# yvette256/nerfstudio-thermal

Measured on AMD Instinct MI355X. Metric: train rays/sec (4096-ray batch, 96 samples/ray), higher is better.
Workload: dtype f32; 1 GPU; thermal-nerfacto density_mode=shared train step (pixel sampling+raygen+fwd+losses+bwd+allreduce+Adam), 4096 rays/GPU, 256/96 proposal + 48 field samples, hash 16x2^19x2 + 2x(5x2^17x2), 8 cameras (4 RGB + 4 thermal); rays_per_gpu=4096, parallelism=dp1, grad_scaler=device-side (optim.DeviceGradScaler)

## Files before the change

### nerfstudio-thermal_amd/csrc/tn_adam.h

```cpp
#pragma once
#include "tn_common.h"

struct AdamCoef {
  float neg_step, bc2_sqrt;
  float b1, b2, omb1, omb2, eps;
};
__host__ __device__ __forceinline__ AdamCoef adam_coef(float neg_step, float bc2_sqrt, double beta1, double beta2, float eps) {
  return AdamCoef{neg_step, bc2_sqrt, (float)beta1, (float)beta2, (float)(1.0 - beta1), (float)(1.0 - beta2), eps};
}
__device__ __forceinline__ void adam1(float& p, float g, float& m, float& v, const AdamCoef& c) {
  const float m_new = m * c.b1 + g * c.omb1;
  const float v_new = v * c.b2 + (c.omb2 * g) * g;
  const float den = sqrtf(v_new) / c.bc2_sqrt + c.eps;
  p = p + c.neg_step * (m_new / den);
  m = m_new;
  v = v_new;
}
#pragma clang fp contract(off)
__device__ __forceinline__ double adam_bias_correction(double beta, int step, int skipped) {
  const int eff = step - skipped;
  return 1.0 - pow(beta, (double)(eff < 1 ? 1 : eff));
}
__device__ __forceinline__ double adam_sched_t(int max_steps, int sched_step, int lag) {
  const double t = (double)(sched_step - lag) / (double)max_steps;
// ... 19 lines not shown
#define TN_FOLD_ADAM_FUSED 1.0f
#define TN_FOLD_ADAM_FELL_BACK 2.0f
struct FoldAdamHost {
  float *p, *m, *v;
  float* state;
  float* found_inf;
  int flag;
  const int32_t* skipped;
  int lag_index;
  int step, max_steps, sched_step;
  double lr, lr_final, beta1, beta2;
  float eps;
  const float* grads;
  int ncheck;
  int64_t check_off[TN_TRAIN_STEP_MAX_RANGES], check_cnt[TN_TRAIN_STEP_MAX_RANGES];
};
```

### nerfstudio-thermal_amd/csrc/tn_common.h

```cpp
#pragma once
#include <hip/hip_runtime.h>
#include <stdint.h>
#include <math.h>
#include "../../include/thermal_nerf_hip.h"

#define TN_WAVE 64

void tn_set_error(const char* fmt, ...);
#define TN_REQUIRE(cond, ...)        \
  do {                               \
    if (!(cond)) {                   \
      tn_set_error(__VA_ARGS__);     \
      return TN_EINVAL;              \
    }                                \
  } while (0)
#define TN_CHECK_LAUNCH(name)                                         \
  do {                                                                \
    hipError_t e__ = hipGetLastError();                               \
    if (e__ != hipSuccess) {                                          \
      tn_set_error("%s: %s", name, hipGetErrorString(e__));           \
      return TN_ELAUNCH;                                              \
    }                                                                 \
  } while (0)

// ... 350 lines not shown
int tn_train_losses_clip(const float* s_bins_fine, const float* weights_fine, int32_t S_fine, int32_t num_props, const float* const* s_bins_prop,
                         const float* const* weights_prop, const int32_t* S_prop, float* const* d_weights_prop, int64_t N, float distortion_mult,
                         float interlevel_mult, float* d_weights_fine, const float* pred_rgb, int32_t rgb_stride, const float* pred_thermal,
                         int32_t thermal_stride, const float* image, const float* is_thermal, float thermal_mult, float tv_mult, float cross_mult,
                         float* d_pred_rgb, float* d_pred_thermal, float* loss_lines, float* depth_expected, const float* scratch, int clip_nblk,
                         tn_stream_t stream);
struct DposArgs;
struct PoseFinishArgs;
struct FoldAdamHost;
int tn_grid_scatter_launch(const TnGrid& grid, const float* origins, const float* directions, const float* e_bins, const float* g_enc, int ld,
                           int64_t N, int S, float* d_origins, float* d_directions, void* scratch, hipStream_t stream, float* dense_sum = nullptr,
                           bool counters_zeroed = false, const DposArgs* cowork = nullptr, const PoseFinishArgs* fold_cowork = nullptr,
                           const FoldAdamHost* fold_adam = nullptr);
bool tn_grid_scatter_takes_cowork(const TnGrid& grid, int64_t P, void* scratch);
bool tn_fold_adam_takes(const TnGrid& grid, int64_t P, void* scratch);
int tn_field_bwd_phase_ex(const TnField* field, const float* origins, const float* directions, const int64_t* camera_indices, const float* e_bins,
                          const float* d_density, const float* d_rgb, int64_t N, int32_t S, void* workspace, int64_t workspace_bytes, float* d_origins,
                          float* d_directions, int32_t phases, int32_t level_begin, int32_t level_end, const PoseFinishArgs* fold_cowork,
                          bool* fold_cowork_taken, tn_stream_t stream, const FoldAdamHost* fold_adam = nullptr);
int tn_pose_finish_args(const float* pose_adjustment, const uint8_t* frozen, const int64_t* camera_indices, const float* directions_in,
                        const float* d_origins, const float* d_directions, int64_t N, int32_t num_cameras, float* grad_pose, const float* loss_lines,
                        float* losses16, float trans_pen, float rot_pen, float scale, float* reg_out, const float* grads, int32_t num_ranges,
                        const int64_t* offsets, const int64_t* counts, const int32_t* flag_index, int32_t num_flags, float* found_inf, int32_t pose_flag,
                        PoseFinishArgs& a);
void tn_grid_scatter_counters(const TnGrid& grid, int64_t P, void* scratch, uint32_t** ptr, int* words);
__device__ __forceinline__ void tn_zero_words(uint32_t* __restrict__ p, int words) {
  if (blockIdx.x == 0 && blockIdx.y == 0)
    for (int i = threadIdx.x; i < words; i += blockDim.x) p[i] = 0u;
}
bool tn_grid_scatter_is_binned(const TnGrid& grid, int64_t P, const void* scratch);
// ... 8 lines not shown
```

### nerfstudio-thermal_amd/csrc/tn_field.hip

```cpp
#include "tn_common.h"
#include "tn_field_dpos.h"
#include <stdlib.h>

typedef float f32x16 __attribute__((ext_vector_type(16)));
typedef float v4f_t __attribute__((ext_vector_type(4)));
#ifndef FRAG_NT
#define FRAG_NT 1
#endif

#define TILE 32
#define FRAG 64

__host__ __device__ __forceinline__ constexpr int RROW(int r, int h) { return (r & 3) + 8 * (r >> 2) + 4 * h; }

struct LayerGeom { int mo, ti; };
__host__ __device__ __forceinline__ constexpr int layer_mo(int l) { return (l == 0 || l == 2 || l == 3) ? 2 : 1; }
__host__ __device__ __forceinline__ constexpr int layer_ti(int l) { return l == 0 ? 1 : 2; }
__host__ __device__ __forceinline__ constexpr int layer_frags(int l) { return layer_mo(l) * layer_ti(l) * 16; }
__host__ __device__ __forceinline__ constexpr int fwd_off(int l) {
  int o = 0;
  for (int i = 0; i < l; ++i) o += layer_frags(i) * FRAG;
  return o;
}
#define PACK_FWD_FLOATS (fwd_off(5))
// ... 770 lines not shown
#define FB_NO_SB 0
#endif
#ifndef FB_TOUCH
#define FB_TOUCH 0
#endif
#define FB_SB() do { if (!FB_NO_SB) __builtin_amdgcn_sched_barrier(0); } while (0)
template <bool DENS_ONLY, bool BF3>
__global__ void __launch_bounds__(256, 1) k_field_bwd_fused(const float* __restrict__ pack, const float* __restrict__ sel, const float* __restrict__ ys,
                                                            const float* __restrict__ d_rgb, const float* __restrict__ d_density,
                                                            const int64_t* __restrict__ cam_idx, int num_images, int64_t P, int S, int C,
                                                            const float* __restrict__ shtab, const float* __restrict__ emb,
                                                            float* __restrict__ cam_bias, int L, int64_t PT,
                                                            const float* __restrict__ encs, const float* __restrict__ h1s,
                                                            const float* __restrict__ hins, const float* __restrict__ hh1s,
                                                            const float* __restrict__ hh2s, float* __restrict__ g_enc, FusedGrads G,
                                                            uint32_t* __restrict__ zero_ptr, int zero_words) {
  extern __shared__ __attribute__((aligned(16))) float lds[];
  tn_zero_words(zero_ptr, zero_words);
  const float* src = pack + PACK_BWD_OFF;
  for (int i = threadIdx.x * 4; i < PACK_BWD_FLOATS; i += blockDim.x * 4) {
    const float* sp = (BF3 && i >= fwd_off(2) && i < fwd_off(4)) ? pack + PACK_BF_BWD_OFF + (i - fwd_off(2)) : src + i;
    *reinterpret_cast<float4*>(lds + i) = *reinterpret_cast<const float4*>(sp);
  }
  __syncthreads();
  const int lane = threadIdx.x & 63, j = lane & 31, h = lane >> 5, wv = threadIdx.x >> 6;
  float* bufY = lds + PACK_BWD_FLOATS + wv * FB_WAVE_FLOATS;
  float* bufX = bufY + FB_TILE_FLOATS;
  float* bufG = bufX + FB_TILE_FLOATS;
  int* bufC = reinterpret_cast<int*>(bufG + 128);
  const int64_t ntiles = tn_cdiv(P, TILE);
  const int64_t wave = (int64_t)blockIdx.x * 4 + wv;
// ... 14 lines not shown
#pragma unroll
  for (int b = 0; b < 4; ++b) { acc4[b] = zero4; acc1[b] = zero4; }
  int emb_cam = -1;
  float emb_sum = 0.0f;
  const int64_t tpw = tn_cdiv(ntiles, nwaves);
  const int64_t tile_begin = wave * tpw;
  const int64_t tile_end = (wave + 1) * tpw < ntiles ? (wave + 1) * tpw : ntiles;
  f32x16 nx0 = zero16, nx1 = zero16;
  FbSmall nsm;
  if (tile_begin < tile_end) {
    nsm = fb_load_small<DENS_ONLY>(tile_begin, tile_begin, j, h, P, S, C, num_images, hins, d_density, sel, ys, d_rgb, cam_idx);
    nx0 = load_frag(DENS_ONLY ? h1s : hh2s, tile_begin, 2, 0, lane);
    nx1 = load_frag(DENS_ONLY ? h1s : hh2s, tile_begin, 2, 1, lane);
  }
  float touch_acc = 0.0f;
  for (int64_t tile = tile_begin; tile < tile_end; ++tile) {
    const int64_t p = tile * TILE + j;
    const bool valid = p < P;
    const int64_t pc = valid ? p : P - 1;
    const FbSmall sm = nsm;
    float tch0 = 0.0f, tch1 = 0.0f, tch2 = 0.0f;
    if (FB_TOUCH && tile + 1 < tile_end) {
      const int64_t tn = tile + 1;
      if (!DENS_ONLY) tch0 = hh1s[(tn * 2 * 4 * 64) * 4 + lane * 32];
      tch1 = h1s[(tn * 2 * 4 * 64) * 4 + lane * 32];
      if (lane < 16) {
        if (!DENS_ONLY) tch2 = hins[(tn * 128) * 4 + lane * 32];
      } else if (lane < 48) {
        const int l = (lane - 16) >> 1;
        if (l < L) tch2 = encs[((int64_t)l * PT + tn * TILE) * 2 + ((lane - 16) & 1) * 32];
// ... 126 lines not shown
    }
    WAVE_LDS_SYNC();
    if (!(FB_ABLATE & 2)) wgrad_tile32<2, 1>(bufY, bufX, j, h, acc0, bs0);
    FB_SB();
    f32x16 de = zero16;
#pragma unroll
    for (int r = 0; r < 16; ++r) de = MFMA(AB(0, 0, 0, r), dh0[r], de);
#pragma unroll
    for (int r = 0; r < 16; ++r) de = MFMA(AB(0, 0, 1, r), dh1[r], de);
    if (valid) {
#pragma unroll
      for (int g = 0; g < 4; ++g) {
        *reinterpret_cast<float2*>(g_enc + (int64_t)(4 * g + 2 * h) * 2 * P + 2 * p) = make_float2(de[4 * g], de[4 * g + 1]);
        *reinterpret_cast<float2*>(g_enc + (int64_t)(4 * g + 2 * h + 1) * 2 * P + 2 * p) = make_float2(de[4 * g + 2], de[4 * g + 3]);
      }
    }
    WAVE_LDS_SYNC();
    touch_acc += (tch0 + tch1) + tch2;
  }
#undef AB
  if (touch_acc == 1.2345678e-30f) cam_bias[0] = touch_acc;
  if (FB_ABLATE & 8) return;
  __syncthreads();
  float* red = lds + PACK_BWD_FLOATS;
  if (!DENS_ONLY) {
    float* esum = red + FB_RED_TOTAL;
    int* ecam = reinterpret_cast<int*>(esum + 4 * 64);
    esum[wv * 64 + lane] = emb_sum;
    if (lane == 0) ecam[wv] = emb_cam;
    __syncthreads();
    if (threadIdx.x < 64) {
      for (int e = 0; e < 4; ++e) {
        const int cam = ecam[e];
        if (cam < 0) continue;
        bool first = true;
        for (int f = 0; f < e; ++f) first = first && (ecam[f] != cam);
// ... 248 lines not shown
             "tn_field_bwd: bad phase set %d", phases);
  TN_REQUIRE(!((phases & TN_BWD_SCATTER) && (phases & (TN_BWD_SCATTER_BIN | TN_BWD_SCATTER_FOLD))), "tn_field_bwd: TN_BWD_SCATTER and its two halves exclude each other");
  if (phases & (TN_BWD_SCATTER | TN_BWD_SCATTER_FOLD))
    TN_REQUIRE(level_begin >= 0 && level_begin < level_end && level_end <= field->grid.num_levels, "tn_field_bwd: bad level range [%d, %d)", level_begin,
               level_end);
  int64_t P = N * (int64_t)S;
  FieldWs ws = ws_layout(workspace, P, 1);
  TN_REQUIRE(workspace_bytes >= ws.bytes, "tn_field_bwd: workspace of %lld bytes, tn_field_workspace_bytes(%lld, 1) = %lld", (long long)workspace_bytes, (long long)P,
             (long long)ws.bytes);
  TN_REQUIRE((2 * ws.PT + P) * 8 < (1ll << 32), "tn_field_bwd: batch too large for the 32-bit lane offsets of the level-major loads");
  hipStream_t st = tn_s(stream);
  const int C = field->num_channels;
  TN_REQUIRE(dens_only || !(phases & TN_BWD_MLP) || field->num_images <= FIELD_MAX_IMAGES,
             "tn_field_bwd: %d cameras, the per-camera sums of the appearance embedding's gradient are sized for %d", field->num_images, FIELD_MAX_IMAGES);
  DposArgs dpos_args{};
  bool dpos_cowork = false;
  if (phases & TN_BWD_MLP) {
    const size_t shmem = FB_LDS_FLOATS * sizeof(float);
    const int grid = (int)std::max<int64_t>(1, std::min<int64_t>(tn_cdiv(tn_cdiv(P, TILE), 4), 256));
    FusedGrads G{field->gw0, field->gb0, field->gw1, field->gb1, field->ghw0, field->ghb0, field->ghw1, field->ghb1, field->ghw2, field->ghb2, field->gemb};
    uint32_t* zp;
    int zw;
    tn_grid_scatter_counters(field->grid, P, ws.scatter, &zp, &zw);
    if (dens_only) {
      (void)hipFuncSetAttribute(reinterpret_cast<const void*>(&k_field_bwd_fused<true, false>), hipFuncAttributeMaxDynamicSharedMemorySize, (int)shmem);
      hipLaunchKernelGGL((k_field_bwd_fused<true, false>), dim3(grid), dim3(256), shmem, st, ws.pack, ws.sel, ws.y, d_rgb, d_density, camera_indices, field->num_images, P, S,
                         C, ws.sh, field->emb, ws.cam_bias, field->grid.num_levels, ws.PT, ws.enc, ws.h1, ws.hin, ws.hh1, ws.hh2, ws.g_enc, G, zp, zw);
    } else if (tn_head_bf16x3()) {
      (void)hipFuncSetAttribute(reinterpret_cast<const void*>(&k_field_bwd_fused<false, true>), hipFuncAttributeMaxDynamicSharedMemorySize, (int)shmem);
      hipLaunchKernelGGL((k_field_bwd_fused<false, true>), dim3(grid), dim3(256), shmem, st, ws.pack, ws.sel, ws.y, d_rgb, d_density, camera_indices, field->num_images, P,
                         S, C, ws.sh, field->emb, ws.cam_bias, field->grid.num_levels, ws.PT, ws.enc, ws.h1, ws.hin, ws.hh1, ws.hh2, ws.g_enc, G, zp, zw);
    } else {
      (void)hipFuncSetAttribute(reinterpret_cast<const void*>(&k_field_bwd_fused<false, false>), hipFuncAttributeMaxDynamicSharedMemorySize, (int)shmem);
      hipLaunchKernelGGL((k_field_bwd_fused<false, false>), dim3(grid), dim3(256), shmem, st, ws.pack, ws.sel, ws.y, d_rgb, d_density, camera_indices, field->num_images, P,
                         S, C, ws.sh, field->emb, ws.cam_bias, field->grid.num_levels, ws.PT, ws.enc, ws.h1, ws.hin, ws.hh1, ws.hh2, ws.g_enc, G, zp, zw);
    }
    if (!dens_only && d_origins == nullptr)
      hipLaunchKernelGGL(k_field_emb_finish, dim3(std::min(field->num_images + 8, 1024)), dim3(256), 0, st, ws.cam_bias,
                         reinterpret_cast<uint32_t*>(ws.cam_bias + (int64_t)FIELD_MAX_IMAGES * 64), field->hw0, field->emb, field->gemb, field->ghw0,
                         field->num_images);
    TN_CHECK_LAUNCH("tn_field_bwd(mlp + weight gradients)");
    if (d_origins != nullptr) {
      dpos_args = DposArgs{origins, directions, e_bins, ws.g_enc, ws.jac, N, S, field->grid.num_levels, ws.PT, d_origins, d_directions,
                           dens_only ? nullptr : ws.cam_bias, reinterpret_cast<uint32_t*>(ws.cam_bias + (int64_t)FIELD_MAX_IMAGES * 64), field->hw0, field->emb,
                           field->gemb, field->ghw0, field->num_images};
      const char* cwe = getenv("TN_DPOS_COWORK");
      dpos_cowork = (phases & TN_BWD_SCATTER) && level_begin == 0 && level_end == field->grid.num_levels && !(cwe && cwe[0] == '0') &&
                    tn_grid_scatter_takes_cowork(field->grid, P, ws.scatter);
      if (!dpos_cowork) {
        hipStream_t side = (phases & TN_BWD_FORK_DPOS) ? tn_fork(st) : nullptr;
        const int64_t tiles = tn_cdiv(P, 32);
        hipLaunchKernelGGL(k_field_dpos, dim3((unsigned)std::min<int64_t>(tn_cdiv(tiles, 4), 256 * 8)), dim3(256), 0, side ? side : st, dpos_args);
      }
      TN_CHECK_LAUNCH("tn_field_bwd(d position)");
    }
  }
  float* sc_do = nullptr;
  float* sc_dd = nullptr;
  if (phases & TN_BWD_SCATTER) {
    TnGrid sub = level_range_grid(field->grid, level_begin, level_end);
    const bool cz = (phases & (TN_BWD_MLP | TN_BWD_COUNTERS_CLEAN)) && level_begin == 0 && level_end == field->grid.num_levels;
    const PoseFinishArgs* fcw = (fold_cowork != nullptr && dpos_cowork) ? fold_cowork : nullptr;
    const FoldAdamHost* fad = (fold_adam != nullptr && dpos_cowork) ? fold_adam : nullptr;
    rc = tn_grid_scatter_launch(sub, origins, directions, e_bins, ws.g_enc + (int64_t)level_begin * 2 * P, TN_LD_LEVEL_MAJOR, N, S, sc_do, sc_dd, ws.scatter, st,
                                nullptr, cz, dpos_cowork ? &dpos_args : nullptr, fcw, fad);
    if (fold_cowork_taken && rc == TN_OK) *fold_cowork_taken = fcw != nullptr;
  }
  if (phases & (TN_BWD_SCATTER_BIN | TN_BWD_SCATTER_FOLD)) {
    TN_REQUIRE(tn_grid_scatter_is_binned(field->grid, P, ws.scatter), "tn_field_bwd: the two-step scatter needs a record-based path (TN_SCATTER_MODE=2 or 1 -- not 0 --, a scatter workspace, table <= 2^20 slots)");
    if (phases & TN_BWD_SCATTER_BIN)
      rc = tn_grid_scatter_bin(field->grid, origins, directions, e_bins, ws.g_enc, TN_LD_LEVEL_MAJOR, N, S, sc_do, sc_dd, ws.scatter, st,
                               (phases & (TN_BWD_MLP | TN_BWD_COUNTERS_CLEAN)) != 0);
    if (rc == TN_OK && (phases & TN_BWD_SCATTER_FOLD)) rc = tn_grid_scatter_fold(field->grid, P, ws.scatter, level_begin, level_end, st);
  }
  if (phases & TN_BWD_JOIN) tn_join_all(st);
  return rc;
}

// ... 38 lines not shown
```

### nerfstudio-thermal_amd/csrc/tn_field_dpos.h

```cpp
#pragma once
#include "tn_common.h"

struct DposArgs {
  const float* origins; const float* directions; const float* e_bins; const float* g_enc; const float* jac;
  int64_t N; int S; int L; int64_t PT;
  float* d_origins; float* d_directions;
  float* cam_bias; uint32_t* fin_counter; const float* hw0; const float* emb; float* gemb; float* ghw0; int num_images;
};

__device__ __forceinline__ void emb_finish_jobs(float* __restrict__ cam_bias, uint32_t* __restrict__ counter, const float* __restrict__ hw0,
                                                const float* __restrict__ emb, float* __restrict__ gemb, float* __restrict__ ghw0, int num_images,
                                                float* sums , int* flag , unsigned bid, unsigned nblk) {
  const int t = threadIdx.x;
  const int njobs = num_images + 8;
  if ((int)bid >= njobs) return;
  const unsigned workers = (unsigned)njobs < nblk ? (unsigned)njobs : nblk;
  for (int job = bid; job < njobs; job += nblk) {
    if (job < num_images) {
      const int cam = job;
      float v = 0.0f;
      if (t < 64) {
        v = cam_bias[(int64_t)cam * 64 + t];
        sums[t] = v;
      }
      __syncthreads();
      if (t < 64 && __ballot(v != 0.0f) != 0ull) {
        const int e = t & 31, half = t >> 5;
        float a = 0.0f;
        for (int f = 0; f < 32; ++f) a += hw0[(32 * half + f) * 63 + 31 + e] * sums[32 * half + f];
        a += __shfl_xor(a, 32, 64);
        if (half == 0 && a != 0.0f) gemb[(int64_t)cam * 32 + e] += a;
      }
      __syncthreads();
    } else {
      const int o = (job - num_images) * 256 + t;
      if (t < 256 && o < 2048) {
        const int f = o >> 5, e = o & 31;
        float a = 0.0f;
        for (int cam = 0; cam < num_images; ++cam) {
          const float b = cam_bias[(int64_t)cam * 64 + f];
          if (b != 0.0f) a += b * emb[(int64_t)cam * 32 + e];
        }
        if (a != 0.0f) ghw0[f * 63 + 31 + e] += a;
      }
    }
  }
  __syncthreads();
  if (t == 0) *flag = (__hip_atomic_fetch_add(counter, 1u, __ATOMIC_RELAXED, __HIP_MEMORY_SCOPE_AGENT) == workers - 1) ? 1 : 0;
  __syncthreads();
  if (*flag) {
    for (int i = t; i < num_images * 64; i += blockDim.x) cam_bias[i] = 0.0f;
    if (t == 0) *counter = 0u;
  }
}

__device__ __forceinline__ void field_dpos_body(const DposArgs& a, unsigned bid, unsigned nblk, float* emb_sums , int* emb_flag) {
  if (a.cam_bias != nullptr) emb_finish_jobs(a.cam_bias, a.fin_counter, a.hw0, a.emb, a.gemb, a.ghw0, a.num_images, emb_sums, emb_flag, bid, nblk);
  const int64_t N = a.N, PT = a.PT;
  const int S = a.S, L = a.L;
  const int64_t P = N * (int64_t)S;
  const int64_t ntiles = tn_cdiv(P, 32);
  const int lane = threadIdx.x & 63, j = lane & 31, h = lane >> 5;
  typedef float v2f_t __attribute__((ext_vector_type(2)));
  for (int64_t tile = (int64_t)bid * (blockDim.x >> 6) + (threadIdx.x >> 6); tile < ntiles; tile += (int64_t)nblk * (blockDim.x >> 6)) {
    const int64_t p = tile * 32 + j;
    const bool live = p < P;
    const int64_t pc = live ? p : P - 1;
    float dx = 0.f, dy = 0.f, dz = 0.f;
#pragma unroll
    for (int q = 0; q < 4; ++q) {
      float2 gl[2];
      v2f_t jl[2][3];
// ... 54 lines not shown
```

### nerfstudio-thermal_amd/csrc/tn_scatter.hip

```cpp
#include "tn_common.h"
#include "tn_field_dpos.h"
#include "tn_pose_finish.h"
#include "tn_adam.h"
#include <float.h>
#include <stdlib.h>
#include <stdio.h>
#include <vector>
#include <algorithm>

__device__ __forceinline__ float seg_sum4(float v, int start, int lane) {
  int sl = lane >> 2;
#pragma unroll
  for (int o = 1; o < 16; o <<= 1) {
    float t = __shfl_up(v, 4 * o, 64);
    if (sl - o >= start) v += t;
  }
  return v;
}

__global__ void __launch_bounds__(256) k_grid_scatter(GridK g, const float* __restrict__ origins, const float* __restrict__ directions,
                                                      const float* __restrict__ e_bins, const float* __restrict__ g_enc, int ld, int64_t N, int S,
                                                      float* __restrict__ d_origins, float* __restrict__ d_directions, int level_groups, ReplicaK rk) {
  const bool want_dpos = d_origins != nullptr;
  const int lane = tn_lane();
// ... 599 lines not shown
  uint16_t* idx;
  float2* val;
  uint32_t* hdr;
  uint32_t NB;
  int slice_log2, nslices;
  uint32_t merge_mask;
  uint32_t segc;
  uint32_t chunks;
  uint32_t* wmax;
};
struct FoldAdamScal {
  float* state;
  const int32_t* skipped;
  int flag, lag_index, step, max_steps, sched_step;
  double lr, lr_final, beta1, beta2;
};
__device__ __forceinline__ void fold_adam_scalars_block(const FoldAdamScal& a, double* s_term ) {
  if ((threadIdx.x & 63) == 0 && threadIdx.x < 256) {
    const int w = threadIdx.x >> 6;
    const int sk = a.skipped ? a.skipped[a.flag] : 0;
    const int lag = (a.skipped != nullptr && a.lag_index >= 0) ? a.skipped[a.lag_index] : 0;
    const double t = a.max_steps > 0 ? adam_sched_t(a.max_steps, a.sched_step, lag) : 0.0;
    if (w < 2) s_term[w] = adam_bias_correction(w == 0 ? a.beta1 : a.beta2, a.step, sk);
    else if (a.max_steps > 0) s_term[w] = adam_log_lr_term(w == 2 ? a.lr : a.lr_final, w == 2 ? 1.0 - t : t);
  }
  __syncthreads();
  if (threadIdx.x == 0) {
    float ns, bc;
    adam_scalars_finish(s_term[0], s_term[1], a.max_steps > 0 ? exp(s_term[2] + s_term[3]) : a.lr, ns, bc);
    a.state[2] = ns;
    a.state[3] = bc;
  }
}
#define SEG_CAP (BIN_THREADS * 8)
#define SEG_REGION (SEG_CAP + TN_BIN_MAX_SLICES)
#ifndef SEG_FOLD_ABLATE
#define SEG_FOLD_ABLATE 0
#endif

template <bool WANT_DPOS>
__global__ void __launch_bounds__(BIN_THREADS, 4) k_seg_bin(GridK g, const float* __restrict__ origins, const float* __restrict__ directions,
                                                         const float* __restrict__ e_bins, const float* __restrict__ g_enc, int ld, int64_t N, int S,
                                                         float* __restrict__ d_origins, float* __restrict__ d_directions, int level_groups, SegK sk,
                                                         DposArgs cw, int cw_blocks, FoldAdamScal fs) {
  __shared__ uint32_t s_cnt[TN_BIN_MAX_SLICES];
  __shared__ uint32_t s_off[TN_BIN_MAX_SLICES + 1];
  __shared__ __attribute__((aligned(16))) uint16_t s_i16[SEG_REGION];
  __shared__ __attribute__((aligned(16))) float2 s_val[SEG_REGION];
  const unsigned bx = blockIdx.x;
  if (!WANT_DPOS && bx >= sk.NB + (unsigned)cw_blocks) {
    if (blockIdx.y == 0) fold_adam_scalars_block(fs, reinterpret_cast<double*>(s_val));
    return;
  }
  if (!WANT_DPOS && bx >= sk.NB) {
    field_dpos_body(cw, blockIdx.y * (unsigned)cw_blocks + (bx - sk.NB), (unsigned)cw_blocks * gridDim.y, reinterpret_cast<float*>(s_val),
                    reinterpret_cast<int*>(s_cnt));
    return;
  }
  const int lane = tn_lane();
  const int tid = threadIdx.x, wv = tid >> 6;
  const int ns = sk.nslices;
  const int64_t P = N * (int64_t)S;
  int64_t i = (int64_t)bx * BIN_THREADS + tid;
  const bool live = i < P;
  if (!live) i = P - 1;
  int64_t ray;
// ... 5 lines not shown
  const float* eb = e_bins + ray * (S + 1) + s;
  const float st = eb[0], en = eb[1];
  const Contracted c = tn_contract(o[0], o[1], o[2], d[0], d[1], d[2], st, en);
  const int nlev = (g.L - (int)blockIdx.y + level_groups - 1) / level_groups;
  constexpr int GVP = WANT_DPOS ? 0 : 5;
  float2 gvp[GVP + 1];
#pragma unroll
  for (int li = 0; li < GVP; ++li) {
    const int l = blockIdx.y + li * level_groups;
    gvp[li] = (live && li < nlev) ? *reinterpret_cast<const float2*>(ld > 0 ? g_enc + p * ld + 2 * l : g_enc + (int64_t)l * 2 * P + 2 * p) : make_float2(0.f, 0.f);
  }
  for (int t = tid; t < ns; t += BIN_THREADS) s_cnt[t] = 0;
  __syncthreads();
  const uint32_t smask = (1u << sk.slice_log2) - 1u;
  float dpx = 0.f, dpy = 0.f, dpz = 0.f;
  uint32_t gmax = 0u;
#pragma unroll 1
  for (int li = 0; li < nlev; ++li) {
    const int l = blockIdx.y + li * level_groups;
    const float res = g.res[l];
    const bool merge = (sk.merge_mask >> l) & 1u;
    BinLevel b;
    bin_level(c, res, g.mask, merge, live, lane, b);
    if (b.emit) {
#pragma unroll
      for (int k = 0; k < 8; ++k) b.idx[k] |= atomicAdd(&s_cnt[b.idx[k] >> sk.slice_log2], 1u) << 20;
    }
    __syncthreads();
    if (wv == (li & (BIN_THREADS / 64 - 1))) {
      uint32_t run = 0;
      uint32_t* hdr = sk.hdr + ((size_t)l * ns) * sk.NB + bx;
// ... 13 lines not shown
          s_cnt[sl] = 0u;
          hdr[(size_t)sl * sk.NB] = off | (cnt << 16);
        }
        run += __shfl(inc, 63, 64);
      }
      if (lane == 0) s_off[ns] = run;
    }
    float2 gv = make_float2(0.f, 0.f);
    if (li < GVP) {
#pragma unroll
      for (int q = 0; q < GVP; ++q)
        if (q == li) gv = gvp[q];
    } else if (live) {
      gv = *reinterpret_cast<const float2*>(ld > 0 ? g_enc + p * ld + 2 * l : g_enc + (int64_t)l * 2 * P + 2 * p);
    }
    if (!WANT_DPOS && fs.state != nullptr) gmax = max(gmax, max(__float_as_uint(gv.x) & 0x7fffffffu, __float_as_uint(gv.y) & 0x7fffffffu));
    if (WANT_DPOS) {
      const float2* tb = g.table + (size_t)l * g.tsize;
      float sk8[8];
#pragma unroll
      for (int k = 0; k < 8; ++k) {
        const float2 t = tb[b.idx[k] & 0xfffffu];
        sk8[k] = gv.x * t.x + gv.y * t.y;
      }
      float ax = 0.f, ay = 0.f, az = 0.f;
#pragma unroll
      for (int v = 0; v < 2; ++v)
#pragma unroll
        for (int u = 0; u < 2; ++u) {
          ax += b.wy[u] * b.wz[v] * (sk8[1 + 2 * u + 4 * v] - sk8[0 + 2 * u + 4 * v]);
          ay += b.wx[u] * b.wz[v] * (sk8[u + 2 + 4 * v] - sk8[u + 0 + 4 * v]);
// ... 19 lines not shown
        s_i16[pos] = (uint16_t)(b.idx[k] & smask);
        s_val[pos] = make_float2(vx[k], vy[k]);
      }
    }
    __syncthreads();
    const uint32_t total = s_off[ns];
    const size_t reg = ((size_t)l * sk.NB + bx) * SEG_REGION;
    {
      float4* __restrict__ dv = reinterpret_cast<float4*>(sk.val + reg);
      const float4* sv = reinterpret_cast<const float4*>(s_val);
      for (uint32_t j = tid; j < (total + 1) / 2; j += BIN_THREADS) dv[j] = sv[j];
      uint4* __restrict__ di = reinterpret_cast<uint4*>(sk.idx + reg);
      const uint4* si = reinterpret_cast<const uint4*>(s_i16);
      for (uint32_t j = tid; j < (total + 7) / 8; j += BIN_THREADS) di[j] = si[j];
    }
  }
  if (!WANT_DPOS && fs.state != nullptr) {
#pragma unroll
    for (int o2 = 32; o2 >= 1; o2 >>= 1) gmax = max(gmax, (uint32_t)__shfl_xor((int)gmax, o2, 64));
    if (lane == 0) sk.wmax[((size_t)blockIdx.y * sk.NB + bx) * (BIN_THREADS / 64) + wv] = gmax;
  }
  if (WANT_DPOS) {
    float wxg, wyg, wzg;
    tn_contract_bwd(c, dpx, dpy, dpz, wxg, wyg, wzg);
    if (!live) { wxg = wyg = wzg = 0.0f; }
    const float tm = (st + en) / 2.0f;
    float v[6] = {wxg, wyg, wzg, wxg * tm, wyg * tm, wzg * tm};
    const int r32 = (int)ray;
    const int lead = __shfl(r32, lane & 3, 64);
    if (__all(r32 == lead)) {
#pragma unroll
      for (int k = 0; k < 6; ++k) {
        float r = v[k];
        r += __shfl_xor(r, 4, 64);
        r += __shfl_xor(r, 8, 64);
// ... 205 lines not shown
    }
#pragma unroll
    for (int u = 0; u < 8; ++u) {
      const uint32_t t = tt + u * FOLD_THREADS + tid;
      if (!nz[u]) continue;
      if (!split) {
        const float2 r = make_float2(cv[u].x + w[u].x, cv[u].y + w[u].y);
        dst[t] = r;
        if (g.nonfinite != nullptr && ((r.x - r.x) + (r.y - r.y)) != 0.0f) *g.nonfinite = 1.0f;
      } else {
        if (w[u].x != 0.0f) unsafeAtomicAdd(reinterpret_cast<float*>(dst + t), w[u].x);
        if (w[u].y != 0.0f) unsafeAtomicAdd(reinterpret_cast<float*>(dst + t) + 1, w[u].y);
        if (g.nonfinite != nullptr && ((w[u].x - w[u].x) + (w[u].y - w[u].y)) != 0.0f) *g.nonfinite = 1.0f;
      }
    }
  }
}

struct FoldAdamPrep {
  const float* grads;
  int ncheck;
  int64_t off[TN_TRAIN_STEP_MAX_RANGES], cnt[TN_TRAIN_STEP_MAX_RANGES];
  float* found_inf_flag;
  float* state;
  float limit;
  const uint32_t* wmax;
  uint32_t row_words, row_stride, rows;
};
__global__ void __launch_bounds__(1024) k_fold_adam_prepare(FoldAdamPrep a) {
  __shared__ int s_bad;
  __shared__ uint32_t s_max;
  if (threadIdx.x == 0) { s_bad = 0; s_max = 0u; }
  __syncthreads();
  bool bad = false;
  for (int k = 0; k < a.ncheck; ++k) {
    const float* base = a.grads + a.off[k];
    for (int64_t i0 = threadIdx.x; i0 < a.cnt[k]; i0 += 8 * (int64_t)blockDim.x) {
      float x[8];
#pragma unroll
      for (int u = 0; u < 8; ++u) { const int64_t i = i0 + u * (int64_t)blockDim.x; x[u] = i < a.cnt[k] ? base[i] : 0.0f; }
#pragma unroll
      for (int u = 0; u < 8; ++u) bad = bad || ((x[u] - x[u]) != 0.0f);
    }
  }
  uint32_t mx = 0u;
  for (uint32_t r = 0; r < a.rows; ++r) {
    const uint32_t* row = a.wmax + (size_t)r * a.row_stride;
    for (uint32_t i0 = threadIdx.x; i0 < a.row_words; i0 += 8 * blockDim.x) {
      uint32_t w[8];
#pragma unroll
      for (int u = 0; u < 8; ++u) { const uint32_t i = i0 + u * blockDim.x; w[u] = i < a.row_words ? row[i] : 0u; }
#pragma unroll
      for (int u = 0; u < 8; ++u) mx = max(mx, w[u]);
    }
  }
#pragma unroll
  for (int o = 32; o >= 1; o >>= 1) mx = max(mx, (uint32_t)__shfl_xor((int)mx, o, 64));
  const bool wave_bad = __any(bad);
  if ((threadIdx.x & 63) == 0) {
    if (wave_bad) s_bad = 1;
    atomicMax(&s_max, mx);
  }
  __syncthreads();
  if (threadIdx.x == 0) {
    if (s_bad) *a.found_inf_flag = 1.0f;
    const float enc_max = __uint_as_float(s_max);
    a.state[0] = enc_max;
    a.state[1] = (enc_max <= a.limit) ? TN_FOLD_ADAM_FUSED : TN_FOLD_ADAM_FELL_BACK;
  }
}

static int env_int(const char* name, int dflt, int lo, int hi) {
  const char* e = getenv(name);
  int v = e ? atoi(e) : dflt;
  return v < lo ? lo : (v > hi ? hi : v);
}
static int dense_replicas() { static int r = env_int("TN_SCATTER_REPLICAS", 16, 0, 64); return r; }

static int64_t plan_replicas(const TnGrid& grid, int64_t P, ReplicaK& rk) {
  const int64_t cap = TN_SCATTER_SCRATCH_BYTES / (int64_t)sizeof(float2);
  const int64_t T = 1ll << grid.log2_hashmap_size;
  int64_t used = 0, total = 0;
  if (dense_replicas() <= 0) return 0;
// ... 113 lines not shown
    const int blocks = (int)sk.NB;
    const int level_groups = seg_level_groups(L, sk.NB);
    TN_REQUIRE(cowork == nullptr || d_origins == nullptr, "tn_grid_scatter: co-work only beside a bin pass without a d position path of its own");
    if (d_origins != nullptr) {
      hipLaunchKernelGGL(k_seg_bin<true>, dim3(blocks, level_groups), dim3(BIN_THREADS), 0, stream, gk, origins, directions, e_bins, g_enc, ld, N, S, d_origins,
                         d_directions, level_groups, sk, DposArgs{}, 0, FoldAdamScal{});
    } else {
      int cw_blocks = 0;
      if (cowork != nullptr) {
        const int64_t tiles = tn_cdiv(cowork->N * (int64_t)cowork->S, 32);
        cw_blocks = (int)std::min<int64_t>(tn_cdiv(tn_cdiv(tiles, BIN_THREADS / 64), level_groups), 2048);
      }
      FoldAdamScal fs{};
      if (fold_adam != nullptr) {
        const FoldAdamHost& h = *fold_adam;
        fs = FoldAdamScal{h.state, h.skipped, h.flag, h.lag_index, h.step, h.max_steps, h.sched_step, h.lr, h.lr_final, h.beta1, h.beta2};
      }
      hipLaunchKernelGGL(k_seg_bin<false>, dim3(blocks + cw_blocks + (fold_adam ? 1 : 0), level_groups), dim3(BIN_THREADS), 0, stream, gk, origins, directions,
                         e_bins, g_enc, ld, N, S, d_origins, d_directions, level_groups, sk, cowork ? *cowork : DposArgs{}, cw_blocks, fs);
    }
    TN_CHECK_LAUNCH("tn_grid_scatter(bin, segmented)");
    return TN_OK;
  }
  TN_REQUIRE(cowork == nullptr, "tn_grid_scatter: co-work needs the segmented path (tn_grid_scatter_takes_cowork)");
  BinK bk;
  uint32_t nblk;
  int rc = bin_plan(grid, P, scratch, bk, nblk);
  if (rc) return rc;
  if (!counters_zeroed) {
    hipError_t e = hipMemsetAsync(bk.count, 0, (size_t)L * bk.nslices * 4 * bk.cstride, stream);
    TN_REQUIRE(e == hipSuccess, "tn_grid_scatter: memset failed: %s", hipGetErrorString(e));
// ... 23 lines not shown
  TN_REQUIRE(level_begin >= 0 && level_begin < level_end && level_end <= L, "tn_grid_scatter_fold: bad level range");
  TN_REQUIRE(cowork == nullptr || seg_mode(), "tn_grid_scatter_fold: co-work needs the segmented path (tn_grid_scatter_takes_cowork)");
  TN_REQUIRE(fold_adam == nullptr || (level_begin == 0 && level_end == L && fold_adam->p == grid.table && tn_fold_adam_takes(grid, P, scratch)),
             "tn_grid_scatter_fold: the fold does not step this table (tn_fold_adam_takes, the whole grid in one launch)");
  if (seg_mode()) {
    SegK sk;
    int rc = seg_plan(grid, P, scratch, sk);
    if (rc) return rc;
    GridK gk = make_gridk(grid);
    const size_t shmem = (size_t)(2u << sk.slice_log2) * sizeof(double) + (size_t)sk.segc * 8 + (FOLD_THREADS / 64) * 4;
    const int max_shmem = (int)((2u << TN_BIN_SLICE_LOG2) * sizeof(double) + 1024 * 8 + (FOLD_THREADS / 64) * 4);
    const uint32_t nblk = (uint32_t)(level_end - level_begin) * (uint32_t)sk.nslices * sk.chunks;
    const uint32_t pfb = cowork ? ((uint32_t)cowork->total_blocks + 7u) & ~7u : 0u;
    if (fold_adam != nullptr) {
      const FoldAdamHost& h = *fold_adam;
      FoldAdamPrep pr{};
      pr.grads = h.grads;
      pr.ncheck = h.ncheck;
      for (int k = 0; k < h.ncheck; ++k) { pr.off[k] = h.check_off[k]; pr.cnt[k] = h.check_cnt[k]; }
      pr.found_inf_flag = h.found_inf + h.flag;
      pr.state = h.state;
      pr.limit = FLT_MAX / (8.0f * (float)P);
      pr.wmax = sk.wmax;
      pr.row_words = sk.NB * (BIN_THREADS / 64); pr.row_stride = pr.row_words; pr.rows = (uint32_t)seg_level_groups(L, sk.NB);
      hipLaunchKernelGGL(k_fold_adam_prepare, dim3(1), dim3(1024), 0, stream, pr);
      TN_CHECK_LAUNCH("tn_grid_scatter(fold: prepare)");
      const AdamCoef c = adam_coef(0.f, 0.f, h.beta1, h.beta2, h.eps);
      FoldAdamK fa{reinterpret_cast<float2*>(h.p), reinterpret_cast<float2*>(h.m), reinterpret_cast<float2*>(h.v), h.state, h.found_inf + h.flag,
                   c.b1, c.b2, c.omb1, c.omb2, c.eps};
      (void)hipFuncSetAttribute(reinterpret_cast<const void*>(&k_seg_fold<true>), hipFuncAttributeMaxDynamicSharedMemorySize, max_shmem);
      hipLaunchKernelGGL(k_seg_fold<true>, dim3(nblk + pfb), dim3(FOLD_THREADS), shmem, stream, gk, sk, (uint32_t)level_begin, (uint32_t)(gk.grad_zero ? 1 : 0),
                         cowork ? *cowork : PoseFinishArgs{}, pfb, fa);
    } else {
      (void)hipFuncSetAttribute(reinterpret_cast<const void*>(&k_seg_fold<false>), hipFuncAttributeMaxDynamicSharedMemorySize, max_shmem);
      hipLaunchKernelGGL(k_seg_fold<false>, dim3(nblk + pfb), dim3(FOLD_THREADS), shmem, stream, gk, sk, (uint32_t)level_begin, (uint32_t)(gk.grad_zero ? 1 : 0),
                         cowork ? *cowork : PoseFinishArgs{}, pfb, FoldAdamK{});
    }
    TN_CHECK_LAUNCH("tn_grid_scatter(fold, segmented)");
    return TN_OK;
  }
  BinK bk;
// ... 36 lines not shown
        for (int k = 0; k < 9; ++k) { if (q[4 + k]) { st[k] += (q[4 + k] - prev) / 100.0; prev = q[4 + k]; } }
      }
      if (n) fprintf(stderr, "  level %2d: %4d active blocks, mean us: setup %.1f passes %.1f flush %.1f; first start %.1f last end %.1f | 1st iteration: passes %.2f %.2f %.2f %.2f retries %.2f %.2f %.2f sync %.2f float-atomics %.2f\n", l, n, a / n, b2 / n, c / n, first, last,
                     st[0] / n, st[1] / n, st[2] / n, st[3] / n, st[4] / n, st[5] / n, st[6] / n, st[7] / n, st[8] / n);
    }
  }
  TN_CHECK_LAUNCH("tn_grid_scatter(fold)");
  return TN_OK;
}

bool tn_grid_scatter_is_binned(const TnGrid& grid, int64_t P, const void* scratch) {
  return scratch != nullptr && scatter_mode() >= 1 && grid.log2_hashmap_size - TN_BIN_SLICE_LOG2 <= 8 && P * 8 < (1ll << 31);
}

bool tn_grid_scatter_takes_cowork(const TnGrid& grid, int64_t P, void* scratch) { return seg_mode() && tn_grid_scatter_is_binned(grid, P, scratch); }
bool tn_fold_adam_takes(const TnGrid& grid, int64_t P, void* scratch) {
  if (!tn_grid_scatter_takes_cowork(grid, P, scratch) || !grid.table_grad_is_zero || grid.log2_hashmap_size < 1) return false;
  SegK sk;
  if (seg_plan(grid, P, scratch, sk) != TN_OK) return false;
  return sk.chunks == 1 && ((uintptr_t)grid.table % 16) == 0;
}

static int grid_scatter_binned(const TnGrid& grid, const float* origins, const float* directions, const float* e_bins, const float* g_enc, int ld,
                               int64_t N, int S, float* d_origins, float* d_directions, void* scratch, hipStream_t stream, bool counters_zeroed,
                               const DposArgs* cowork, const PoseFinishArgs* fold_cowork, const FoldAdamHost* fold_adam) {
  int rc = tn_grid_scatter_bin(grid, origins, directions, e_bins, g_enc, ld, N, S, d_origins, d_directions, scratch, stream, counters_zeroed, cowork, fold_adam);
  if (rc) return rc;
  return tn_grid_scatter_fold(grid, N * (int64_t)S, scratch, 0, grid.num_levels, stream, fold_cowork, fold_adam);
}

// ... 102 lines not shown
```

Before: 6.113 million rays/s.

## Compute fold-Adam enc-grad max in MLP bwd and drop separate prepare kernel

```diff
diff --git a/nerfstudio-thermal_amd/csrc/tn_adam.h b/nerfstudio-thermal_amd/csrc/tn_adam.h
--- a/nerfstudio-thermal_amd/csrc/tn_adam.h
+++ b/nerfstudio-thermal_amd/csrc/tn_adam.h
@@ -57,4 +57,6 @@
   const float* grads;
   int ncheck;
   int64_t check_off[TN_TRAIN_STEP_MAX_RANGES], check_cnt[TN_TRAIN_STEP_MAX_RANGES];
+  const uint32_t* enc_wmax;
+  int enc_words;
 };
diff --git a/nerfstudio-thermal_amd/csrc/tn_common.h b/nerfstudio-thermal_amd/csrc/tn_common.h
--- a/nerfstudio-thermal_amd/csrc/tn_common.h
+++ b/nerfstudio-thermal_amd/csrc/tn_common.h
@@ -388,6 +388,7 @@
                            const FoldAdamHost* fold_adam = nullptr);
 bool tn_grid_scatter_takes_cowork(const TnGrid& grid, int64_t P, void* scratch);
 bool tn_fold_adam_takes(const TnGrid& grid, int64_t P, void* scratch);
+uint32_t* tn_fold_adam_enc_words(const TnGrid& grid, int64_t P, void* scratch, int64_t* capacity);
 int tn_field_bwd_phase_ex(const TnField* field, const float* origins, const float* directions, const int64_t* camera_indices, const float* e_bins,
                           const float* d_density, const float* d_rgb, int64_t N, int32_t S, void* workspace, int64_t workspace_bytes, float* d_origins,
                           float* d_directions, int32_t phases, int32_t level_begin, int32_t level_end, const PoseFinishArgs* fold_cowork,
diff --git a/nerfstudio-thermal_amd/csrc/tn_field.hip b/nerfstudio-thermal_amd/csrc/tn_field.hip
--- a/nerfstudio-thermal_amd/csrc/tn_field.hip
+++ b/nerfstudio-thermal_amd/csrc/tn_field.hip
@@ -1,5 +1,6 @@
 #include "tn_common.h"
 #include "tn_field_dpos.h"
+#include "tn_adam.h"
 #include <stdlib.h>
 
 typedef float f32x16 __attribute__((ext_vector_type(16)));
@@ -808,7 +809,7 @@
                                                             const float* __restrict__ encs, const float* __restrict__ h1s,
                                                             const float* __restrict__ hins, const float* __restrict__ hh1s,
                                                             const float* __restrict__ hh2s, float* __restrict__ g_enc, FusedGrads G,
-                                                            uint32_t* __restrict__ zero_ptr, int zero_words) {
+                                                            uint32_t* __restrict__ zero_ptr, int zero_words, uint32_t* __restrict__ enc_wmax) {
   extern __shared__ __attribute__((aligned(16))) float lds[];
   tn_zero_words(zero_ptr, zero_words);
   const float* src = pack + PACK_BWD_OFF;
@@ -853,6 +854,7 @@
     nx1 = load_frag(DENS_ONLY ? h1s : hh2s, tile_begin, 2, 1, lane);
   }
   float touch_acc = 0.0f;
+  uint32_t emax = 0u;
   for (int64_t tile = tile_begin; tile < tile_end; ++tile) {
     const int64_t p = tile * TILE + j;
     const bool valid = p < P;
@@ -1009,12 +1011,20 @@
         *reinterpret_cast<float2*>(g_enc + (int64_t)(4 * g + 2 * h) * 2 * P + 2 * p) = make_float2(de[4 * g], de[4 * g + 1]);
         *reinterpret_cast<float2*>(g_enc + (int64_t)(4 * g + 2 * h + 1) * 2 * P + 2 * p) = make_float2(de[4 * g + 2], de[4 * g + 3]);
       }
+#pragma unroll
+      for (int r = 0; r < 16; ++r)
+        if (4 * (r >> 2) + 2 * h + ((r >> 1) & 1) < L) emax = max(emax, __float_as_uint(de[r]) & 0x7fffffffu);
     }
     WAVE_LDS_SYNC();
     touch_acc += (tch0 + tch1) + tch2;
   }
 #undef AB
   if (touch_acc == 1.2345678e-30f) cam_bias[0] = touch_acc;
+  if (enc_wmax != nullptr) {
+#pragma unroll
+    for (int o = 32; o >= 1; o >>= 1) emax = max(emax, (uint32_t)__shfl_xor((int)emax, o, 64));
+    if (lane == 0) enc_wmax[wave] = emax;
+  }
   if (FB_ABLATE & 8) return;
   __syncthreads();
   float* red = lds + PACK_BWD_FLOATS;
@@ -1293,10 +1303,25 @@
   TN_REQUIRE(dens_only || !(phases & TN_BWD_MLP) || field->num_images <= FIELD_MAX_IMAGES,
              "tn_field_bwd: %d cameras, the per-camera sums of the appearance embedding's gradient are sized for %d", field->num_images, FIELD_MAX_IMAGES);
   DposArgs dpos_args{};
-  bool dpos_cowork = false;
+  const char* cwe = getenv("TN_DPOS_COWORK");
+  const bool dpos_cowork = (phases & TN_BWD_MLP) && d_origins != nullptr && (phases & TN_BWD_SCATTER) && level_begin == 0 &&
+                           level_end == field->grid.num_levels && !(cwe && cwe[0] == '0') && tn_grid_scatter_takes_cowork(field->grid, P, ws.scatter);
+  FoldAdamHost fad_local{};
+  const FoldAdamHost* fad = nullptr;
+  uint32_t* enc_wmax = nullptr;
+  const int mlp_blocks = (int)std::max<int64_t>(1, std::min<int64_t>(tn_cdiv(tn_cdiv(P, TILE), 4), 256));
+  if (fold_adam != nullptr && dpos_cowork) {
+    int64_t cap = 0;
+    enc_wmax = tn_fold_adam_enc_words(field->grid, P, ws.scatter, &cap);
+    TN_REQUIRE(enc_wmax != nullptr && 4 * (int64_t)mlp_blocks <= cap, "tn_field_bwd: the fold does not step this table (tn_fold_adam_takes)");
+    fad_local = *fold_adam;
+    fad_local.enc_wmax = enc_wmax;
+    fad_local.enc_words = 4 * mlp_blocks;
+    fad = &fad_local;
+  }
   if (phases & TN_BWD_MLP) {
     const size_t shmem = FB_LDS_FLOATS * sizeof(float);
-    const int grid = (int)std::max<int64_t>(1, std::min<int64_t>(tn_cdiv(tn_cdiv(P, TILE), 4), 256));
+    const int grid = mlp_blocks;
     FusedGrads G{field->gw0, field->gb0, field->gw1, field->gb1, field->ghw0, field->ghb0, field->ghw1, field->ghb1, field->ghw2, field->ghb2, field->gemb};
     uint32_t* zp;
     int zw;
@@ -1304,15 +1329,15 @@
     if (dens_only) {
       (void)hipFuncSetAttribute(reinterpret_cast<const void*>(&k_field_bwd_fused<true, false>), hipFuncAttributeMaxDynamicSharedMemorySize, (int)shmem);
       hipLaunchKernelGGL((k_field_bwd_fused<true, false>), dim3(grid), dim3(256), shmem, st, ws.pack, ws.sel, ws.y, d_rgb, d_density, camera_indices, field->num_images, P, S,
-                         C, ws.sh, field->emb, ws.cam_bias, field->grid.num_levels, ws.PT, ws.enc, ws.h1, ws.hin, ws.hh1, ws.hh2, ws.g_enc, G, zp, zw);
+                         C, ws.sh, field->emb, ws.cam_bias, field->grid.num_levels, ws.PT, ws.enc, ws.h1, ws.hin, ws.hh1, ws.hh2, ws.g_enc, G, zp, zw, enc_wmax);
     } else if (tn_head_bf16x3()) {
       (void)hipFuncSetAttribute(reinterpret_cast<const void*>(&k_field_bwd_fused<false, true>), hipFuncAttributeMaxDynamicSharedMemorySize, (int)shmem);
       hipLaunchKernelGGL((k_field_bwd_fused<false, true>), dim3(grid), dim3(256), shmem, st, ws.pack, ws.sel, ws.y, d_rgb, d_density, camera_indices, field->num_images, P,
-                         S, C, ws.sh, field->emb, ws.cam_bias, field->grid.num_levels, ws.PT, ws.enc, ws.h1, ws.hin, ws.hh1, ws.hh2, ws.g_enc, G, zp, zw);
+                         S, C, ws.sh, field->emb, ws.cam_bias, field->grid.num_levels, ws.PT, ws.enc, ws.h1, ws.hin, ws.hh1, ws.hh2, ws.g_enc, G, zp, zw, enc_wmax);
     } else {
       (void)hipFuncSetAttribute(reinterpret_cast<const void*>(&k_field_bwd_fused<false, false>), hipFuncAttributeMaxDynamicSharedMemorySize, (int)shmem);
       hipLaunchKernelGGL((k_field_bwd_fused<false, false>), dim3(grid), dim3(256), shmem, st, ws.pack, ws.sel, ws.y, d_rgb, d_density, camera_indices, field->num_images, P,
-                         S, C, ws.sh, field->emb, ws.cam_bias, field->grid.num_levels, ws.PT, ws.enc, ws.h1, ws.hin, ws.hh1, ws.hh2, ws.g_enc, G, zp, zw);
+                         S, C, ws.sh, field->emb, ws.cam_bias, field->grid.num_levels, ws.PT, ws.enc, ws.h1, ws.hin, ws.hh1, ws.hh2, ws.g_enc, G, zp, zw, enc_wmax);
     }
     if (!dens_only && d_origins == nullptr)
       hipLaunchKernelGGL(k_field_emb_finish, dim3(std::min(field->num_images + 8, 1024)), dim3(256), 0, st, ws.cam_bias,
@@ -1322,10 +1347,7 @@
     if (d_origins != nullptr) {
       dpos_args = DposArgs{origins, directions, e_bins, ws.g_enc, ws.jac, N, S, field->grid.num_levels, ws.PT, d_origins, d_directions,
                            dens_only ? nullptr : ws.cam_bias, reinterpret_cast<uint32_t*>(ws.cam_bias + (int64_t)FIELD_MAX_IMAGES * 64), field->hw0, field->emb,
-                           field->gemb, field->ghw0, field->num_images};
-      const char* cwe = getenv("TN_DPOS_COWORK");
-      dpos_cowork = (phases & TN_BWD_SCATTER) && level_begin == 0 && level_end == field->grid.num_levels && !(cwe && cwe[0] == '0') &&
-                    tn_grid_scatter_takes_cowork(field->grid, P, ws.scatter);
+                           field->gemb, field->ghw0, field->num_images, fad ? fad->found_inf + fad->flag : nullptr};
       if (!dpos_cowork) {
         hipStream_t side = (phases & TN_BWD_FORK_DPOS) ? tn_fork(st) : nullptr;
         const int64_t tiles = tn_cdiv(P, 32);
@@ -1340,7 +1362,6 @@
     TnGrid sub = level_range_grid(field->grid, level_begin, level_end);
     const bool cz = (phases & (TN_BWD_MLP | TN_BWD_COUNTERS_CLEAN)) && level_begin == 0 && level_end == field->grid.num_levels;
     const PoseFinishArgs* fcw = (fold_cowork != nullptr && dpos_cowork) ? fold_cowork : nullptr;
-    const FoldAdamHost* fad = (fold_adam != nullptr && dpos_cowork) ? fold_adam : nullptr;
     rc = tn_grid_scatter_launch(sub, origins, directions, e_bins, ws.g_enc + (int64_t)level_begin * 2 * P, TN_LD_LEVEL_MAJOR, N, S, sc_do, sc_dd, ws.scatter, st,
                                 nullptr, cz, dpos_cowork ? &dpos_args : nullptr, fcw, fad);
     if (fold_cowork_taken && rc == TN_OK) *fold_cowork_taken = fcw != nullptr;
diff --git a/nerfstudio-thermal_amd/csrc/tn_field_dpos.h b/nerfstudio-thermal_amd/csrc/tn_field_dpos.h
--- a/nerfstudio-thermal_amd/csrc/tn_field_dpos.h
+++ b/nerfstudio-thermal_amd/csrc/tn_field_dpos.h
@@ -6,11 +6,13 @@
   int64_t N; int S; int L; int64_t PT;
   float* d_origins; float* d_directions;
   float* cam_bias; uint32_t* fin_counter; const float* hw0; const float* emb; float* gemb; float* ghw0; int num_images;
+  float* emb_nonfinite;
 };
 
 __device__ __forceinline__ void emb_finish_jobs(float* __restrict__ cam_bias, uint32_t* __restrict__ counter, const float* __restrict__ hw0,
                                                 const float* __restrict__ emb, float* __restrict__ gemb, float* __restrict__ ghw0, int num_images,
-                                                float* sums , int* flag , unsigned bid, unsigned nblk) {
+                                                float* sums , int* flag , unsigned bid, unsigned nblk,
+                                                float* __restrict__ nonfinite = nullptr) {
   const int t = threadIdx.x;
   const int njobs = num_images + 8;
   if ((int)bid >= njobs) return;
@@ -29,7 +31,11 @@
         float a = 0.0f;
         for (int f = 0; f < 32; ++f) a += hw0[(32 * half + f) * 63 + 31 + e] * sums[32 * half + f];
         a += __shfl_xor(a, 32, 64);
-        if (half == 0 && a != 0.0f) gemb[(int64_t)cam * 32 + e] += a;
+        if (half == 0 && a != 0.0f) {
+          const float r = gemb[(int64_t)cam * 32 + e] + a;
+          gemb[(int64_t)cam * 32 + e] = r;
+          if (nonfinite != nullptr && (r - r) != 0.0f) *nonfinite = 1.0f;
+        }
       }
       __syncthreads();
     } else {
@@ -41,7 +47,11 @@
           const float b = cam_bias[(int64_t)cam * 64 + f];
           if (b != 0.0f) a += b * emb[(int64_t)cam * 32 + e];
         }
-        if (a != 0.0f) ghw0[f * 63 + 31 + e] += a;
+        if (a != 0.0f) {
+          const float r = ghw0[f * 63 + 31 + e] + a;
+          ghw0[f * 63 + 31 + e] = r;
+          if (nonfinite != nullptr && (r - r) != 0.0f) *nonfinite = 1.0f;
+        }
       }
     }
   }
@@ -55,7 +65,7 @@
 }
 
 __device__ __forceinline__ void field_dpos_body(const DposArgs& a, unsigned bid, unsigned nblk, float* emb_sums , int* emb_flag) {
-  if (a.cam_bias != nullptr) emb_finish_jobs(a.cam_bias, a.fin_counter, a.hw0, a.emb, a.gemb, a.ghw0, a.num_images, emb_sums, emb_flag, bid, nblk);
+  if (a.cam_bias != nullptr) emb_finish_jobs(a.cam_bias, a.fin_counter, a.hw0, a.emb, a.gemb, a.ghw0, a.num_images, emb_sums, emb_flag, bid, nblk, a.emb_nonfinite);
   const int64_t N = a.N, PT = a.PT;
   const int S = a.S, L = a.L;
   const int64_t P = N * (int64_t)S;
diff --git a/nerfstudio-thermal_amd/csrc/tn_scatter.hip b/nerfstudio-thermal_amd/csrc/tn_scatter.hip
--- a/nerfstudio-thermal_amd/csrc/tn_scatter.hip
+++ b/nerfstudio-thermal_amd/csrc/tn_scatter.hip
@@ -637,8 +637,43 @@
   const int32_t* skipped;
   int flag, lag_index, step, max_steps, sched_step;
   double lr, lr_final, beta1, beta2;
+  const float* grads;
+  int ncheck;
+  int64_t off[TN_TRAIN_STEP_MAX_RANGES], cnt[TN_TRAIN_STEP_MAX_RANGES];
+  float* found_inf_flag;
+  float limit;
+  const uint32_t* wmax;
+  int words;
 };
-__device__ __forceinline__ void fold_adam_scalars_block(const FoldAdamScal& a, double* s_term ) {
+__device__ __forceinline__ void fold_adam_scalars_block(const FoldAdamScal& a, double* s_term , uint32_t* s_red ) {
+  if (threadIdx.x == 0) { s_red[0] = 0u; s_red[1] = 0u; }
+  __syncthreads();
+  bool bad = false;
+  for (int k = 0; k < a.ncheck; ++k) {
+    const float* base = a.grads + a.off[k];
+    for (int64_t i0 = threadIdx.x; i0 < a.cnt[k]; i0 += 8 * (int64_t)blockDim.x) {
+      float x[8];
+#pragma unroll
+      for (int u = 0; u < 8; ++u) { const int64_t i = i0 + u * (int64_t)blockDim.x; x[u] = i < a.cnt[k] ? base[i] : 0.0f; }
+#pragma unroll
+      for (int u = 0; u < 8; ++u) bad = bad || ((x[u] - x[u]) != 0.0f);
+    }
+  }
+  uint32_t mx = 0u;
+  for (int i0 = threadIdx.x; i0 < a.words; i0 += 8 * (int)blockDim.x) {
+    uint32_t w[8];
+#pragma unroll
+    for (int u = 0; u < 8; ++u) { const int i = i0 + u * (int)blockDim.x; w[u] = i < a.words ? a.wmax[i] : 0u; }
+#pragma unroll
+    for (int u = 0; u < 8; ++u) mx = max(mx, w[u]);
+  }
+#pragma unroll
+  for (int o = 32; o >= 1; o >>= 1) mx = max(mx, (uint32_t)__shfl_xor((int)mx, o, 64));
+  const bool wave_bad = __any(bad);
+  if ((threadIdx.x & 63) == 0) {
+    if (wave_bad) s_red[1] = 1u;
+    atomicMax(&s_red[0], mx);
+  }
   if ((threadIdx.x & 63) == 0 && threadIdx.x < 256) {
     const int w = threadIdx.x >> 6;
     const int sk = a.skipped ? a.skipped[a.flag] : 0;
@@ -653,6 +688,10 @@
     adam_scalars_finish(s_term[0], s_term[1], a.max_steps > 0 ? exp(s_term[2] + s_term[3]) : a.lr, ns, bc);
     a.state[2] = ns;
     a.state[3] = bc;
+    if (s_red[1]) *a.found_inf_flag = 1.0f;
+    const float enc_max = __uint_as_float(s_red[0]);
+    a.state[0] = enc_max;
+    a.state[1] = (enc_max <= a.limit) ? TN_FOLD_ADAM_FUSED : TN_FOLD_ADAM_FELL_BACK;
   }
 }
 #define SEG_CAP (BIN_THREADS * 8)
@@ -672,7 +711,7 @@
   __shared__ __attribute__((aligned(16))) float2 s_val[SEG_REGION];
   const unsigned bx = blockIdx.x;
   if (!WANT_DPOS && bx >= sk.NB + (unsigned)cw_blocks) {
-    if (blockIdx.y == 0) fold_adam_scalars_block(fs, reinterpret_cast<double*>(s_val));
+    if (blockIdx.y == 0) fold_adam_scalars_block(fs, reinterpret_cast<double*>(s_val), s_cnt);
     return;
   }
   if (!WANT_DPOS && bx >= sk.NB) {
@@ -708,7 +747,6 @@
   __syncthreads();
   const uint32_t smask = (1u << sk.slice_log2) - 1u;
   float dpx = 0.f, dpy = 0.f, dpz = 0.f;
-  uint32_t gmax = 0u;
 #pragma unroll 1
   for (int li = 0; li < nlev; ++li) {
     const int l = blockIdx.y + li * level_groups;
@@ -752,7 +790,6 @@
     } else if (live) {
       gv = *reinterpret_cast<const float2*>(ld > 0 ? g_enc + p * ld + 2 * l : g_enc + (int64_t)l * 2 * P + 2 * p);
     }
-    if (!WANT_DPOS && fs.state != nullptr) gmax = max(gmax, max(__float_as_uint(gv.x) & 0x7fffffffu, __float_as_uint(gv.y) & 0x7fffffffu));
     if (WANT_DPOS) {
       const float2* tb = g.table + (size_t)l * g.tsize;
       float sk8[8];
@@ -802,11 +839,6 @@
       const uint4* si = reinterpret_cast<const uint4*>(s_i16);
       for (uint32_t j = tid; j < (total + 7) / 8; j += BIN_THREADS) di[j] = si[j];
     }
-  }
-  if (!WANT_DPOS && fs.state != nullptr) {
-#pragma unroll
-    for (int o2 = 32; o2 >= 1; o2 >>= 1) gmax = max(gmax, (uint32_t)__shfl_xor((int)gmax, o2, 64));
-    if (lane == 0) sk.wmax[((size_t)blockIdx.y * sk.NB + bx) * (BIN_THREADS / 64) + wv] = gmax;
   }
   if (WANT_DPOS) {
     float wxg, wyg, wzg;
@@ -1042,59 +1074,6 @@
         if (g.nonfinite != nullptr && ((w[u].x - w[u].x) + (w[u].y - w[u].y)) != 0.0f) *g.nonfinite = 1.0f;
       }
     }
-  }
-}
-
-struct FoldAdamPrep {
-  const float* grads;
-  int ncheck;
-  int64_t off[TN_TRAIN_STEP_MAX_RANGES], cnt[TN_TRAIN_STEP_MAX_RANGES];
-  float* found_inf_flag;
-  float* state;
-  float limit;
-  const uint32_t* wmax;
-  uint32_t row_words, row_stride, rows;
-};
-__global__ void __launch_bounds__(1024) k_fold_adam_prepare(FoldAdamPrep a) {
-  __shared__ int s_bad;
-  __shared__ uint32_t s_max;
-  if (threadIdx.x == 0) { s_bad = 0; s_max = 0u; }
-  __syncthreads();
-  bool bad = false;
-  for (int k = 0; k < a.ncheck; ++k) {
-    const float* base = a.grads + a.off[k];
-    for (int64_t i0 = threadIdx.x; i0 < a.cnt[k]; i0 += 8 * (int64_t)blockDim.x) {
-      float x[8];
-#pragma unroll
-      for (int u = 0; u < 8; ++u) { const int64_t i = i0 + u * (int64_t)blockDim.x; x[u] = i < a.cnt[k] ? base[i] : 0.0f; }
-#pragma unroll
-      for (int u = 0; u < 8; ++u) bad = bad || ((x[u] - x[u]) != 0.0f);
-    }
-  }
-  uint32_t mx = 0u;
-  for (uint32_t r = 0; r < a.rows; ++r) {
-    const uint32_t* row = a.wmax + (size_t)r * a.row_stride;
-    for (uint32_t i0 = threadIdx.x; i0 < a.row_words; i0 += 8 * blockDim.x) {
-      uint32_t w[8];
-#pragma unroll
-      for (int u = 0; u < 8; ++u) { const uint32_t i = i0 + u * blockDim.x; w[u] = i < a.row_words ? row[i] : 0u; }
-#pragma unroll
-      for (int u = 0; u < 8; ++u) mx = max(mx, w[u]);
-    }
-  }
-#pragma unroll
-  for (int o = 32; o >= 1; o >>= 1) mx = max(mx, (uint32_t)__shfl_xor((int)mx, o, 64));
-  const bool wave_bad = __any(bad);
-  if ((threadIdx.x & 63) == 0) {
-    if (wave_bad) s_bad = 1;
-    atomicMax(&s_max, mx);
-  }
-  __syncthreads();
-  if (threadIdx.x == 0) {
-    if (s_bad) *a.found_inf_flag = 1.0f;
-    const float enc_max = __uint_as_float(s_max);
-    a.state[0] = enc_max;
-    a.state[1] = (enc_max <= a.limit) ? TN_FOLD_ADAM_FUSED : TN_FOLD_ADAM_FELL_BACK;
   }
 }
 
@@ -1238,7 +1217,16 @@
       FoldAdamScal fs{};
       if (fold_adam != nullptr) {
         const FoldAdamHost& h = *fold_adam;
+        TN_REQUIRE(h.enc_wmax == sk.wmax && h.enc_words >= 0 && h.enc_words <= TN_MAX_LEVELS * (int64_t)sk.NB * (BIN_THREADS / 64),
+                   "tn_grid_scatter: the fold steps its table from the d enc maxima of tn_fold_adam_enc_words");
         fs = FoldAdamScal{h.state, h.skipped, h.flag, h.lag_index, h.step, h.max_steps, h.sched_step, h.lr, h.lr_final, h.beta1, h.beta2};
+        fs.grads = h.grads;
+        fs.ncheck = h.ncheck;
+        for (int k = 0; k < h.ncheck; ++k) { fs.off[k] = h.check_off[k]; fs.cnt[k] = h.check_cnt[k]; }
+        fs.found_inf_flag = h.found_inf + h.flag;
+        fs.limit = FLT_MAX / (8.0f * (float)P);
+        fs.wmax = h.enc_wmax;
+        fs.words = h.enc_words;
       }
       hipLaunchKernelGGL(k_seg_bin<false>, dim3(blocks + cw_blocks + (fold_adam ? 1 : 0), level_groups), dim3(BIN_THREADS), 0, stream, gk, origins, directions,
                          e_bins, g_enc, ld, N, S, d_origins, d_directions, level_groups, sk, cowork ? *cowork : DposArgs{}, cw_blocks, fs);
@@ -1292,17 +1280,6 @@
     const uint32_t pfb = cowork ? ((uint32_t)cowork->total_blocks + 7u) & ~7u : 0u;
     if (fold_adam != nullptr) {
       const FoldAdamHost& h = *fold_adam;
-      FoldAdamPrep pr{};
-      pr.grads = h.grads;
-      pr.ncheck = h.ncheck;
-      for (int k = 0; k < h.ncheck; ++k) { pr.off[k] = h.check_off[k]; pr.cnt[k] = h.check_cnt[k]; }
-      pr.found_inf_flag = h.found_inf + h.flag;
-      pr.state = h.state;
-      pr.limit = FLT_MAX / (8.0f * (float)P);
-      pr.wmax = sk.wmax;
-      pr.row_words = sk.NB * (BIN_THREADS / 64); pr.row_stride = pr.row_words; pr.rows = (uint32_t)seg_level_groups(L, sk.NB);
-      hipLaunchKernelGGL(k_fold_adam_prepare, dim3(1), dim3(1024), 0, stream, pr);
-      TN_CHECK_LAUNCH("tn_grid_scatter(fold: prepare)");
       const AdamCoef c = adam_coef(0.f, 0.f, h.beta1, h.beta2, h.eps);
       FoldAdamK fa{reinterpret_cast<float2*>(h.p), reinterpret_cast<float2*>(h.m), reinterpret_cast<float2*>(h.v), h.state, h.found_inf + h.flag,
                    c.b1, c.b2, c.omb1, c.omb2, c.eps};
@@ -1369,6 +1346,13 @@
 }
 
 bool tn_grid_scatter_takes_cowork(const TnGrid& grid, int64_t P, void* scratch) { return seg_mode() && tn_grid_scatter_is_binned(grid, P, scratch); }
+uint32_t* tn_fold_adam_enc_words(const TnGrid& grid, int64_t P, void* scratch, int64_t* capacity) {
+  SegK sk;
+  *capacity = 0;
+  if (!tn_fold_adam_takes(grid, P, scratch) || seg_plan(grid, P, scratch, sk) != TN_OK) return nullptr;
+  *capacity = TN_MAX_LEVELS * (int64_t)sk.NB * (BIN_THREADS / 64);
+  return sk.wmax;
+}
 bool tn_fold_adam_takes(const TnGrid& grid, int64_t P, void* scratch) {
   if (!tn_grid_scatter_takes_cowork(grid, P, scratch) || !grid.table_grad_is_zero || grid.log2_hashmap_size < 1) return false;
   SegK sk;
```

After: 6.162 million rays/s (median of 6 runs). About the same (+0.8%).
